# flexcompute/tidy3d

Measured on AMD Instinct MI355X. Metric: Mcells/s on 512^3 Yee grid, higher is better.
Workload: dtype f32; 1 GPU; v0: vacuum, PEC walls, curl stencil only; 512^3 Yee cells, Ez point dipole (GaussianPulse 200 THz), random +-1e-3 initial fields; parallelism=z-slab x1, bytes_per_cell_step=72

## Files before the change

### tidy3d_amd/csrc/fdtd_fused2.hpp

```cpp
#pragma once
#include "fdtd_kernels.hpp"

namespace fdtd {

constexpr int kMaxInj = 256;
struct InjP {
  int n;
  const int* start;
  const int4* ent;
  const float* val;
  const float* val2;
  int e2_in_sweep;
  float* cap;
  const int* dstart;
  const int* dlist;
  const struct DumpBox* dboxes;
  float* dump;
};
struct DumpBox {
  int lo0, lo1, lo2, nx, ny, nz;
  int off[6];
};
constexpr int kMaxDumps = 8;
struct DampT {
// ... 93 lines not shown
        if (!fused2_instantiated(fused2_lb(W, opt), opt)) return false;
        const int rep = fused2_opt(nt, mat, mon, clip, damp, disp, src, wv, true, W);
        if (!clip && fused2_rep_word(opt) && !fused2_instantiated(fused2_lb(W, rep), rep)) return false;
      }
    }
  return true;
}
static_assert(fused2_words_instantiated(), "fused2_opt forms a word that no list of instantiations holds");

#if !defined(FDTD_NO_EXJ)
#define FDTD_NO_EXJ 0
#endif
constexpr bool fused2_exj(int lb, int opt) { return !FDTD_NO_EXJ && (opt & kF2Damp) == 0 && !(lb == 512 && (opt & kF2Mat) != 0); }
constexpr int fused2_xch_arrays(int lb, int opt) {
  const int wv = fused2_whatif(opt);
  if (wv) return wv == 13 ? 9 : ((wv >= 10 && wv <= 12) ? 6 + (wv == 11 ? 2 : 3) : 8);
  return fused2_exj(lb, opt) ? 9 : 8;
}
constexpr size_t fused2_lds_bytes(int lb, int opt, int waves) {
  return ((size_t)fused2_xch_arrays(lb, opt) * waves * 64 + ((opt & kF2Damp) ? 2 * 64 : 0)) * sizeof(float4) + ((opt & kF2Mat) ? (size_t)kMaxMedia * sizeof(float2) : 0);
}
static_assert(fused2_lds_bytes(1024, kF2NT | kF2Mat | kF2Mon | kF2Clip | kF2Disp | kF2Src, 16) <= 160 * 1024 && fused2_lds_bytes(1024, kF2Mat | kF2Damp, 16) <= 160 * 1024 &&
              2 * fused2_lds_bytes(512, kF2NT, 8) <= 160 * 1024 && 2 * fused2_lds_bytes(512, kF2Mat | kF2Damp, 8) <= 160 * 1024,
              "fused2_step_kernel: LDS of a workgroup (two per CU for eight waves)");
constexpr bool fused2_lds_pinned(int lb, int opt) {
  const int wv = fused2_whatif(opt), w = lb / 64;
  if (wv) return fused2_lds_bytes(lb, opt, 16) == ((size_t)(wv == 13 ? 9 : ((wv >= 10 && wv <= 12) ? 6 + (wv == 11 ? 2 : 3) : 8)) * 16 * 64) * sizeof(float4);
  return fused2_lds_bytes(lb, opt, w) == ((size_t)(fused2_exj(lb, opt) ? 9 : 8) * w * 64 + ((opt & 8) ? 2 * 64 : 0)) * sizeof(float4) + ((opt & 2) ? (size_t)kMaxMedia * sizeof(float2) : 0);
}
#define FDTD_F2_X(LBV, OV) && fused2_lds_pinned(LBV, OV)
static_assert(true FDTD_F2_LIST_ALL(FDTD_F2_X), "fused2_lds_bytes: the LDS of a listed instantiation changed");
#undef FDTD_F2_X
constexpr int kMaxCap = 1024;
constexpr int kSeamArrays = 13;

void launch_inject_values(hipStream_t st, float* val, const float* w_re, const float* w_im, const float2* wave,
                          long long step, int n);
struct Fused2Launch {
  hipStream_t st;
  int waves, opt, grid_blocks;
  GridP g; FieldP a, b; StepP s; MatP m;
  int zchunk, nbx, nby, nbz, xcd_remap;
  InjP inj; float* seam; DampT dmp; ClipP clip; TileClassP tcl; DispP dp; SrcP sr;
};
#define FDTD_F2_ARGS(L) (L).g, (L).a, (L).b, (L).s, (L).m, (L).zchunk, (L).nbx, (L).nby, (L).nbz, (L).xcd_remap, (L).inj, (L).seam, (L).dmp, (L).clip, (L).tcl, (L).dp, (L).sr
#define FDTD_F2_CASE(LBV, OV)                                                                                                      \
  case fused2_key(LBV, OV):                                                                                                        \
    hipLaunchKernelGGL((fused2_step_kernel<LBV, OV>), dim3(L.grid_blocks, 1, 1), dim3(64, L.waves, 1), fused2_lds_bytes(LBV, OV, L.waves), L.st, \
                       FDTD_F2_ARGS(L));                                                                                           \
    return true;
#define FDTD_F2_LAUNCHER(NAME, LIST)                                                                                               \
  bool NAME(const Fused2Launch& L) {                                                                                               \
    switch (fused2_key(fused2_lb(L.waves, L.opt), L.opt)) { LIST(FDTD_F2_CASE) default: return false; }                            \
  }
bool launch_fused2_step(const Fused2Launch& L);
bool launch_fused2_step_src(const Fused2Launch& L);
bool launch_fused2_step_whatif(const Fused2Launch& L);
bool launch_fused2_step_disp(const Fused2Launch& L);
bool launch_fused2_step_clip(const Fused2Launch& L);
void launch_inject_table(hipStream_t st, float* tab, long long stride, long long off, const float* w_re, const float* w_im,
                         const float2* wave, long long n_steps, int n);
constexpr int kPairMons = 4;
struct PairRecP {
  int n_mon;
  int pre_done;
  BoxP box[kPairMons];
  int nc[kPairMons];
  int comp[kPairMons][6];
  int cap_off[kPairMons];
  float* out_n[kPairMons];
  float* out_m[kPairMons];
};
void launch_pair_record(hipStream_t st, const PairRecP& r, long long max_cells, const GridP& g, const FieldP& a, const FieldP& b,
                        const float* cap);
struct DftDumpP { int n; int slot[3]; int off[3]; };
void launch_dft_record_dump(hipStream_t st, const DftDumpP& r, const float* dump, float2* acc, long long cells, long long fstride,
                            const float2* phase, int nf);
void launch_seams(hipStream_t st, const GridP& g, const FieldP& b, const StepP& s, const MatP& m, const float* seam,
                  int n_seams, const DampT& dmp, const ClipP& clip, const InjP& inj, const SrcP& sr = SrcP{}, float* rep = nullptr);
constexpr int kRepArraysHost = 7;
inline size_t seam_scratch_floats(const GridP& g, int n_tiles_x) { return (size_t)n_tiles_x * kSeamArrays * (size_t)(g.nz + 2) * (size_t)g.ny; }
inline size_t seam_rep_floats(const GridP& g, int n_tiles_x) { return (size_t)n_tiles_x * kRepArraysHost * (size_t)g.nz * (size_t)g.ny; }
void launch_seam_flush(hipStream_t st, const GridP& g, const FieldP& b, const float* rep, int n_seams);

}
```

### tidy3d_amd/csrc/fdtd_kernels2.hpp

```cpp
#pragma once
#include "fdtd_fused2.hpp"

namespace fdtd {

__global__ __launch_bounds__(256) void pair_record_kernel(PairRecP r, GridP g, FieldP a, FieldP b, const float* cap) {
  const int mi = blockIdx.y / 6, ic = blockIdx.y % 6;
  if (mi >= r.n_mon || ic >= r.nc[mi]) return;
  const BoxP bx = r.box[mi];
  const long long cells = (long long)bx.nx * bx.ny * bx.nz;
  const long long t = (long long)blockIdx.x * blockDim.x + threadIdx.x;
  if (t >= cells) return;
  const int c = r.comp[mi][ic];
  const int lx = (int)(t % bx.nx), ly = (int)((t / bx.nx) % bx.ny), lz = (int)(t / ((long long)bx.nx * bx.ny));
  const long long p = (long long)(bx.lo2 + lz) * g.sxy + (long long)(bx.lo1 + ly) * g.nx + bx.lo0 + lx;
  const long long idx = (long long)ic * cells + t;
  const float* fa = c == 0 ? a.ex : (c == 1 ? a.ey : (c == 2 ? a.ez : (c == 3 ? a.hx : (c == 4 ? a.hy : a.hz))));
  const float* fb = c == 0 ? b.ex : (c == 1 ? b.ey : (c == 2 ? b.ez : (c == 3 ? b.hx : (c == 4 ? b.hy : b.hz))));
  const float mid = cap[r.cap_off[mi] + idx];
  float* on = r.out_n[mi];
  float* om = r.out_m[mi];
  if (c < 3) {
    if (on && !r.pre_done) on[idx] = 1.0f * fa[p];
    if (om) om[idx] = 1.0f * mid;
  } else {
// ... 6 lines not shown
                                                              long long fstride, const float2* phase, int nf) {
  const int q = blockIdx.y;
  const long long t = (long long)blockIdx.x * blockDim.x + threadIdx.x;
  if (t >= cells || q >= r.n) return;
  const float v = dump[r.off[q] + t];
  float2* a0 = acc + (long long)r.slot[q] * cells;
  for (int k = 0; k < nf; ++k) {
    const float2 ph = phase[k];
    float2 a = a0[(long long)k * fstride + t];
    a.x += v * ph.x;
    a.y += v * ph.y;
    a0[(long long)k * fstride + t] = a;
  }
}

__global__ __launch_bounds__(256) void inject_table_kernel(float* tab, long long stride, long long off, const float* w_re,
                                                           const float* w_im, const float2* wave, long long n_steps, int n) {
  const long long g = (long long)blockIdx.x * blockDim.x + threadIdx.x;
  if (g >= n_steps * n) return;
  const long long step = g / n;
  const int t = (int)(g % n);
  const float2 a = wave[step];
  tab[step * stride + off + t] = w_re[t] * a.x - w_im[t] * a.y;
}

__global__ __launch_bounds__(256) void inject_values_kernel(float* val, const float* w_re, const float* w_im,
                                                            const float2* wave, long long step, int n) {
  const int t = threadIdx.x;
  if (t >= n) return;
  const float2 a = wave[step];
  val[t] = w_re[t] * a.x - w_im[t] * a.y;
}

__device__ __forceinline__ long long seam_at(const GridP& g, int seam, int arr, int j, int k) {
  return (((long long)seam * kSeamArrays + arr) * (g.nz + 2) + (k + 1)) * g.ny + j;
}

constexpr int kRepArrays = 7;
__device__ __forceinline__ long long rep_base(const GridP& g, int n_tiles_x) {
  return (long long)n_tiles_x * kSeamArrays * (g.nz + 2) * g.ny;
}
__device__ __forceinline__ long long rep_at(const GridP& g, int seam, int arr, int j, int k) {
  return (((long long)seam * kRepArrays + arr) * g.nz + k) * g.ny + j;
}

__device__ __forceinline__ float lane_next(float v) {
#if defined(__HIP_DEVICE_COMPILE__)
  const int x = __builtin_bit_cast(int, v);
  return __builtin_bit_cast(float, __builtin_amdgcn_update_dpp(x, x, 0x130, 0xf, 0xf, false));
#else
  return __shfl_down(v, 1);
#endif
}
__device__ __forceinline__ float lane_prev(float v) {
#if defined(__HIP_DEVICE_COMPILE__)
  const int x = __builtin_bit_cast(int, v);
  return __builtin_bit_cast(float, __builtin_amdgcn_update_dpp(x, x, 0x138, 0xf, 0xf, false));
#else
  return __shfl_up(v, 1);
#endif
}

__device__ __forceinline__ void lds_dma16(const float* base, unsigned off, float4* dst, int lane) {
#if defined(__HIP_DEVICE_COMPILE__)
  const unsigned lds_addr = __builtin_amdgcn_readfirstlane((unsigned)(size_t)dst);
  unsigned keep;
  asm volatile("s_mov_b32 %0, m0\n\ts_mov_b32 m0, %2\n\ts_nop 0\n\tglobal_load_lds_dwordx4 %1, %3\n\ts_mov_b32 m0, %0"
               : "=&s"(keep) : "v"(off), "s"(lds_addr), "s"(base) : "memory");
#else
  dst[lane] = *reinterpret_cast<const float4*>(reinterpret_cast<const char*>(base) + off);
#endif
}
__device__ __forceinline__ void lds_dma_wait() {
// ... 154 lines not shown
    float ezx = lane_next(ezm[0]);
    if (act && (tx == 63 || last_x)) ezx = last_x ? (per_x ? a.ez[pb] : 0.f) : a.ez[pb + ux + V];
    const float ipz = s.ipz[kA - 1];
    ldf<V, true>(ho, uni(a.hx + pb), ubc);
    ldf<V, true>(hoy, uni(a.hy + pb), ubc);
    if constexpr (REP) {
      if (act && tx == 63 && !last_x) {
        const float* r = rpl + (long long)(kA - 1) * g.ny;
        hoy[V - 1] = r[0]; exm[V - 1] = r[2 * rep_arr]; eym[V - 1] = r[3 * rep_arr]; ezm[V - 1] = r[4 * rep_arr]; ezx = r[6 * rep_arr];
        if (use_jp) ezj[V - 1] = r[4 * rep_arr + 1];
      }
      if (xh) {
        const float* r = rpr + (long long)(kA - 1) * g.ny;
        eym[0] = r[5 * rep_arr]; ezm[0] = r[6 * rep_arr];
        if (use_jp) ezj[0] = r[6 * rep_arr + 1];
      }
    }
    if constexpr (DAMP) {
      const float czp = dmp.fc[2][kA - 1];
      const float4 b4 = xdm[tx], c4 = xdm[64 + tx];
      const float bx[V] = {b4.x, b4.y, b4.z, b4.w}, cx[V] = {c4.x, c4.y, c4.z, c4.w};
#pragma unroll
      for (int e = 0; e < V; ++e) { ho[e] *= bx[e] * cyv * czp; hoy[e] *= cx[e] * byv * czp; }
    }
#pragma unroll
    for (int e = 0; e < V; ++e) h1x[e] = upd_h(ho[e], ch, ezj[e] - ezm[e], ipy, eyk[e] - eym[e], ipz);
#pragma unroll
    for (int e = 0; e < V; ++e) {
      const float ez_ip = (e + 1 < V) ? ezm[(e + 1) % V] : ezx;
      h1y[e] = upd_h(hoy[e], ch, exk[e] - exm[e], ipz, ez_ip - ezm[e], ipx[e]);
    }
  }
  int cur = 0;
  const long long seam_arr = (long long)(g.nz + 2) * g.ny;
  const long long seam_row = seam_at(g, tile_x, 0, j, 0);
  struct Ld {
    float exn[V], eyn[V], ezk[V], exj[V], ezj[V], hxn[V], hyn[V], hzn[V];
    float eyx_g, ezx_g;
    float exn_m, ez_mm, ey_mm, ex_jm, hy_o, hz_o;
  };
  [[maybe_unused]] float4* pfb = xch + NXCH * slot;
  [[maybe_unused]] auto pf_issue = [&](int k) __attribute__((always_inline)) {
    if constexpr (PF != 0) {
      const long long pb = (long long)k * g.sxy + rowb;
      const long long up = (k < g.nz) ? g.sxy : 0;
      lds_dma_fence();
      if constexpr (PF == 10) {
        lds_dma16(uni(a.hx + pb), ubc, pfb + 0 * slot + ty * 64, tx);
        lds_dma16(uni(a.hy + pb), ubc, pfb + 1 * slot + ty * 64, tx);
        lds_dma16(uni(a.hz + pb), ubc, pfb + 2 * slot + ty * 64, tx);
      } else if constexpr (PF == 11) {
        lds_dma16(uni(a.ey + pb + up), ubc, pfb + 0 * slot + ty * 64, tx);
        lds_dma16(uni(a.hy + pb), ubc, pfb + 1 * slot + ty * 64, tx);
      } else {
        lds_dma16(uni(a.ex + pb + up), ubc, pfb + 0 * slot + ty * 64, tx);
        lds_dma16(uni(a.ey + pb + up), ubc, pfb + 1 * slot + ty * 64, tx);
        lds_dma16(uni(a.ez + pb), ubc, pfb + 2 * slot + ty * 64, tx);
      }
    }
  };
  [[maybe_unused]] auto pf_take = [&](int q, float (&o)[V]) __attribute__((always_inline)) {
    const float4 t4 = pfb[q * slot + me];
    o[0] = t4.x; o[1] = t4.y; o[2] = t4.z; o[3] = t4.w;
  };
  auto issue = [&](int k, Ld& L) __attribute__((always_inline)) {
    if constexpr (WHATIF == 3) {
      if (ty < 2 || ty == W - 1) {
        zero<V>(L.exn); zero<V>(L.eyn); zero<V>(L.ezk); zero<V>(L.exj); zero<V>(L.ezj); zero<V>(L.hxn); zero<V>(L.hyn); zero<V>(L.hzn);
// ... 60 lines not shown
            L.ezj[V - 1] = r[4 * rep_arr + 1];
            if (!EXJ || ty == W - 1 || k == kA) L.exj[V - 1] = r[2 * rep_arr + 1];
          }
        }
        if (xh) {
          const float* r = rpr + (long long)k * g.ny;
          L.ezk[0] = r[6 * rep_arr];
          if (up1) L.eyn[0] = r[5 * rep_arr + g.ny];
          if (use_jp) L.ezj[0] = r[6 * rep_arr + 1];
          if (do_e1) {
            L.exn_m = up1 ? r[2 * rep_arr + g.ny] : a.ex[pb + im + up];
            L.ez_mm = r[4 * rep_arr]; L.ey_mm = r[3 * rep_arr];
            if (use_jp) L.ex_jm = r[2 * rep_arr + 1];
            L.hy_o = r[0]; L.hz_o = r[rep_arr];
          }
        }
      }
    }
    if constexpr (PF != 0) {
      lds_dma_wait();
      if constexpr (PF == 10) { pf_take(0, L.hxn); pf_take(1, L.hyn); pf_take(2, L.hzn); }
      else if constexpr (PF == 11) { pf_take(0, L.eyn); pf_take(1, L.hyn); }
      else { pf_take(0, L.exn); pf_take(1, L.eyn); pf_take(2, L.ezk); }
    }
  };
  Ld LA, LB2;
  auto body = [&](int k, Ld& L) __attribute__((always_inline)) {
    const int txo = (MAT || DAMP) ? tx : opaque_lane(tx);
    const int i0o = (tile_x * 64 + txo) * V;
    const bool act = i0o < g.nx, last_x = i0o + V >= g.nx, first_x = i0o == 0;
    const bool xh = act && txo == 0 && (!first_x || per_x);
    [[maybe_unused]] const bool wall_x0 = first_x && !pmc_x0 && !per_x;
    const bool seam_l = (txo == 63 && !last_x) || (per_x && last_x), seam_r = txo == 0 && (tile_x > 0 || per_x);
    const long long seam_back = (tile_x > 0 ? -1 : (long long)(nbx - 1)) * kSeamArrays * seam_arr;
    const long long pb = (long long)k * g.sxy + rowb;
    const float ipz = s.ipz[k], idz = s.idz[k];
    [[maybe_unused]] float bzk = 1.f, czk = 1.f;
    if constexpr (DAMP) { bzk = dmp.fb[2][min(k, g.nz - 1)]; czk = dmp.fc[2][min(k, g.nz - 1)]; }
    int q0 = 0, q1 = 0;
    if (inj.n > 0) { q0 = inj.start[k]; q1 = inj.start[k + 1]; }
    [[maybe_unused]] int d0 = 0, d1 = 0;
    if constexpr (MON) { if (inj.dstart) { d0 = inj.dstart[k]; d1 = inj.dstart[k + 1]; } }
    float hy_m = 0.f, hz_m = 0.f;
    float (&exn)[V] = L.exn, (&eyn)[V] = L.eyn, (&ezk)[V] = L.ezk, (&exj)[V] = L.exj, (&ezj)[V] = L.ezj;
    float (&hxn)[V] = L.hxn, (&hyn)[V] = L.hyn, (&hzn)[V] = L.hzn;
    [[maybe_unused]] uint32_t rw = kBgWord;
    if constexpr (MAT) {
      if (do_e1) rw = m.roww[((long long)min(k, g.nz - 1) * g.ny + j) * nbx + tile_x];
    }
    [[maybe_unused]] int ss = -1;
    if constexpr (SRC) {
      if (do_e1 && k < g.nz) ss = sr.sseg[((long long)k * g.ny + j) * nbx + tile_x];
    }
    [[maybe_unused]] int ds = -1;
    if constexpr (DISP) {
      if (do_e1 && k < g.nz) ds = dp.dseg[((long long)k * g.ny + j) * nbx + tile_x];
    }
    if constexpr (WHATIF == 7) {
      issue(k, L);
      if (own && k > k0 && act) {
        const long long po = pb - g.sxy + i0;
        float o0[V], o1[V], o2[V];
#pragma unroll
        for (int e = 0; e < V; ++e) { o0[e] = L.exn[e] + L.exj[e]; o1[e] = L.ezk[e] + L.ezj[e]; o2[e] = L.eyn[e]; }
        stv_h<V, NT>(b.ex + po, o0); stv_h<V, NT>(b.ey + po, o2); stv_h<V, NT>(b.ez + po, o1);
        stv_h<V, NT>(b.hx + po, L.hxn); stv_h<V, NT>(b.hy + po, L.hyn); stv_h<V, NT>(b.hz + po, L.hzn);
      }
// ... 195 lines not shown
                  hit &= hit - 1;
                  const int d = lane_value(ev.x, l) - i0, c = lane_value(ev.z, l) - 8, w = lane_value(ev.w, l);
#pragma unroll
                  for (int e = 0; e < V; ++e)
                    if (d == e) inj.cap[w] = c == 0 ? e1xn[e] : (c == 1 ? e1yn[e] : e1zn[e]);
                }
              }
            }
          }
        }
        if constexpr (MON) {
          if (own && k >= k0 && k < k1) {
            for (int q = d0; q < d1; ++q) {
              const DumpBox bx = inj.dboxes[inj.dlist[q]];
              const int ly = j - bx.lo1, lz = k - bx.lo2;
              if (ly >= 0 && ly < bx.ny) {
                const long long rowo = ((long long)lz * bx.ny + ly) * bx.nx;
#pragma unroll
                for (int e = 0; e < V; ++e) {
                  const int lx = i0o + e - bx.lo0;
                  if (lx >= 0 && lx < bx.nx && act && (!CLIP || (i0o + e >= clip.i0 && i0o + e < clip.i1))) {
                    if (bx.off[0] >= 0) inj.dump[bx.off[0] + rowo + lx] = e1xn[e];
                    if (bx.off[1] >= 0) inj.dump[bx.off[1] + rowo + lx] = e1yn[e];
                    if (bx.off[2] >= 0) inj.dump[bx.off[2] + rowo + lx] = e1zn[e];
                    if (bx.off[3] >= 0) inj.dump[bx.off[3] + rowo + lx] = hxn[e];
                    if (bx.off[4] >= 0) inj.dump[bx.off[4] + rowo + lx] = hyn[e];
                    if (bx.off[5] >= 0) inj.dump[bx.off[5] + rowo + lx] = hzn[e];
                  }
                }
              }
            }
          }
        }
        if (WHATIF != 9 && (CLIP || (own && k >= k0 && k < k1)) && act) {
          float* sp = seam + seam_row + (long long)k * g.ny;
          if (seam_l) {
            sp[0] = hyn[V - 1];
            sp[seam_arr] = hzn[V - 1];
            sp[2 * seam_arr] = e1xn[V - 1];
            sp[3 * seam_arr] = e1yn[V - 1];
            sp[4 * seam_arr] = e1zn[V - 1];
          }
          if (seam_r) {
            sp[5 * seam_arr + seam_back] = e1yn[0];
            sp[6 * seam_arr + seam_back] = e1zn[0];
          }
        }
      }
    }
    float h2x[V], h2y[V], h2z[V];
    unspecified<V>(h2x); unspecified<V>(h2y); unspecified<V>(h2z);
    if (do_h2 && k > kA) {
      if constexpr (DAMP) {
        {
          const float4 b4 = xdm[tx];
          const float bx[V] = {b4.x, b4.y, b4.z, b4.w};
#pragma unroll
          for (int e = 0; e < V; ++e) h1x[e] *= bx[e] * cyv * cz_m;
        }
        {
          const float4 c4 = xdm[64 + tx];
          const float cx[V] = {c4.x, c4.y, c4.z, c4.w};
#pragma unroll
          for (int e = 0; e < V; ++e) { h1y[e] *= cx[e] * byv * cz_m; h1z[e] *= cx[e] * cyv * bz_m; }
        }
      }
      if constexpr (SRC) {
        if (ss_m >= 0 && act && sr.t->use_h2) {
          const long long qs = ((long long)ss_m * 3) * 256 + tx * V;
          float tx_[V], ty_[V], tz_[V];
          ldv<V>(tx_, sr.t->h2 + qs); ldv<V>(ty_, sr.t->h2 + qs + 256); ldv<V>(tz_, sr.t->h2 + qs + 512);
#pragma unroll
          for (int e = 0; e < V; ++e) { h1x[e] = h1x[e] + tx_[e]; h1y[e] = h1y[e] + ty_[e]; h1z[e] = h1z[e] + tz_[e]; }
          if (sr.t->h2b) {
            ldv<V>(tx_, sr.t->h2b + qs); ldv<V>(ty_, sr.t->h2b + qs + 256); ldv<V>(tz_, sr.t->h2b + qs + 512);
#pragma unroll
            for (int e = 0; e < V; ++e) { h1x[e] = h1x[e] + tx_[e]; h1y[e] = h1y[e] + ty_[e]; h1z[e] = h1z[e] + tz_[e]; }
          }
        }
// ... 11 lines not shown
              const float v = inj.val2[lane_value(ev.w, l)];
#pragma unroll
              for (int e = 0; e < V; ++e) {
                const bool mine = d == e;
                h1x[e] = (mine && code == 3) ? h1x[e] + v : h1x[e];
                h1y[e] = (mine && code == 4) ? h1y[e] + v : h1y[e];
                h1z[e] = (mine && code == 5) ? h1z[e] + v : h1z[e];
              }
            }
          }
        }
      }
      float eyx = lane_next(e1y[0]);
      float ezx = lane_next(e1z[0]);
      if (txo == 63 || last_x) { eyx = 0.f; ezx = 0.f; }
      float4 t0, t1;
      if constexpr (WHATIF == 6) {
        t0 = make_float4(e1x[0], e1x[1], e1x[2], e1x[3]); t1 = make_float4(e1z[0], e1z[1], e1z[2], e1z[3]);
      } else {
        t0 = xch[(4 + (E1S ? 0 : (cur ^ 1) * 2) + 0) * slot + me + 64];
        t1 = xch[(4 + (E1S ? 0 : (cur ^ 1) * 2) + 1) * slot + me + 64];
      }
      const float exj1[V] = {t0.x, t0.y, t0.z, t0.w}, ezj1[V] = {t1.x, t1.y, t1.z, t1.w};
#pragma unroll
      for (int e = 0; e < V; ++e) {
        const float ey_ip = (e + 1 < V) ? e1y[(e + 1) % V] : eyx;
        const float ez_ip = (e + 1 < V) ? e1z[(e + 1) % V] : ezx;
        h2x[e] = upd_h(h1x[e], ch, ezj1[e] - e1z[e], ipy, e1yn[e] - e1y[e], ipz_m);
        h2y[e] = upd_h(h1y[e], ch, e1xn[e] - e1x[e], ipz_m, ez_ip - e1z[e], ipx[e]);
        h2z[e] = upd_h(h1z[e], ch, ey_ip - e1y[e], ipx[e], exj1[e] - e1x[e], ipy);
      }
      if constexpr (CLIP) {
        if (act) {
          float* sq = seam + seam_row + (long long)(k - 1) * g.ny;
          if (seam_l) {
            sq[7 * seam_arr] = h2x[V - 1];
            sq[8 * seam_arr] = h2y[V - 2];
            sq[9 * seam_arr] = h2z[V - 2];
          }
          if (seam_r) {
            sq[10 * seam_arr + seam_back] = h2x[0];
            sq[11 * seam_arr + seam_back] = h2y[0];
            sq[12 * seam_arr + seam_back] = h2z[0];
          }
        }
      }
    }
    if constexpr (WHATIF != 6) {
      float4 t4;
      if constexpr (!E1S) {
        t4.x = e1xn[0]; t4.y = e1xn[1]; t4.z = e1xn[2]; t4.w = e1xn[3];
        xch[(4 + cur * 2 + 0) * slot + me] = t4;
        t4.x = e1zn[0]; t4.y = e1zn[1]; t4.z = e1zn[2]; t4.w = e1zn[3];
        xch[(4 + cur * 2 + 1) * slot + me] = t4;
      }
      if constexpr (EXJ) {
        t4.x = exn[0]; t4.y = exn[1]; t4.z = exn[2]; t4.w = exn[3];
        xch[XE * slot + me] = t4;
      }
      if constexpr (EZL) {
        if (k + 1 <= k1) {
          t4.x = ezn_pre[0]; t4.y = ezn_pre[1]; t4.z = ezn_pre[2]; t4.w = ezn_pre[3];
          xch[XZ * slot + me] = t4;
        }
      }
      t4.x = h2x[0]; t4.y = h2x[1]; t4.z = h2x[2]; t4.w = h2x[3];
      xch[2 * slot + me] = t4;
      t4.x = h2z[0]; t4.y = h2z[1]; t4.z = h2z[2]; t4.w = h2z[3];
      xch[3 * slot + me] = t4;
    }
    if constexpr (WHATIF != 2 && WHATIF != 6 && WHATIF != 8) __syncthreads();
    if constexpr (E1S) {
      float4 t4;
      t4.x = e1xn[0]; t4.y = e1xn[1]; t4.z = e1xn[2]; t4.w = e1xn[3];
      xch[4 * slot + me] = t4;
      t4.x = e1zn[0]; t4.y = e1zn[1]; t4.z = e1zn[2]; t4.w = e1zn[3];
// ... 77 lines not shown
          while (hit) {
            const int l = __ffsll(hit) - 1;
            hit &= hit - 1;
            const int d = lane_value(ev.x, l) - i0, code = lane_value(ev.z, l);
            const float v = inj.val2[lane_value(ev.w, l)];
#pragma unroll
            for (int e = 0; e < V; ++e) {
              if (d == e) {
                if (code == 0) ex[e] += v;
                else if (code == 1) ey[e] += v;
                else ez[e] += v;
              }
            }
          }
        }
      }
      if constexpr (DAMP) {
        if (dmp.e2) {
          {
            const float4 c4 = xdm[64 + tx];
            const float cx[V] = {c4.x, c4.y, c4.z, c4.w};
#pragma unroll
            for (int e = 0; e < V; ++e) ex[e] *= cx[e] * byv * bz_m;
          }
          {
            const float4 b4 = xdm[tx];
            const float bx[V] = {b4.x, b4.y, b4.z, b4.w};
#pragma unroll
            for (int e = 0; e < V; ++e) { ey[e] *= bx[e] * cyv * bz_m; ez[e] *= bx[e] * byv * cz_m; }
          }
        }
      }
      if (act && (!CLIP || (i0o >= clip.i0 && i0o < clip.i1))) {
        float* sq = seam + seam_row + (long long)(k - 1) * g.ny;
        if (!CLIP && WHATIF != 9 && txo == 63 && !last_x) {
          sq[7 * seam_arr] = h2x[V - 1];
          sq[8 * seam_arr] = h2y[V - 2];
          sq[9 * seam_arr] = h2z[V - 2];
        }
        if (!CLIP && WHATIF != 9 && txo == 0 && tile_x > 0) {
          sq[10 * seam_arr - kSeamArrays * seam_arr] = h2x[0];
          sq[11 * seam_arr - kSeamArrays * seam_arr] = h2y[0];
          sq[12 * seam_arr - kSeamArrays * seam_arr] = h2z[0];
        }
        const long long po = pb - g.sxy + i0;
        if (WHATIF != 5 || ex[0] == 3.0e38f) {
          stv_h<V, NT>(b.hx + po, h2x);
          stv_h<V, NT>(b.hy + po, h2y);
          stv_h<V, NT>(b.hz + po, h2z);
          stv_h<V, NT>(b.ex + po, ex);
          stv_h<V, NT>(b.ey + po, ey);
          stv_h<V, NT>(b.ez + po, ez);
        }
      }
    }
#pragma unroll
    for (int e = 0; e < V; ++e) {
      h2xm[e] = h2x[e]; h2ym[e] = h2y[e];
      h1x[e] = hxn[e]; h1y[e] = hyn[e]; h1z[e] = hzn[e];
      e1x[e] = e1xn[e]; e1y[e] = e1yn[e]; e1z[e] = e1zn[e];
      exk[e] = exn[e]; eyk[e] = eyn[e];
    }
    exk_m = L.exn_m;
    ipz_m = ipz; idz_m = idz;
    qm0 = q0; qm1 = q1;
    if constexpr (DAMP) { bz_m = bzk; cz_m = czk; }
    if constexpr (MAT) rw_m = rw;
    if constexpr (SRC) ss_m = ss;
    cur ^= 1;
  };
  if constexpr (PF != 0) pf_issue(kA);
  for (int k = kA; k <= k1; k += 2) {
    body(k, LA);
    if (k + 1 <= k1) body(k + 1, LB2);
  }
}
// ... 34 lines not shown
    const int G = xcd_remap, full = total / (8 * G) * (8 * G);
    if (t < full) {
      const int x = t & 7, mloc = t >> 3;
      t = ((mloc / G) * 8 + x) * G + mloc % G;
    }
    if (t >= total) return;
  }
  constexpr int OPTK = OPT | (fused2_exj(LB, OPT) ? 0 : kF2NoExj);
  if constexpr ((OPT & kF2Src) != 0) {
    if (tcl.cls && !(tcl.cls[t] & 4)) {
      fused2_tile_by_class<LB, (OPTK & ~kF2Src)>(g, a, b, s, m, zchunk, nbx, nby, nbz, inj, seam, dmp, clip, t, dp, sr, tcl);
      return;
    }
  }
  fused2_tile_by_class<LB, OPTK>(g, a, b, s, m, zchunk, nbx, nby, nbz, inj, seam, dmp, clip, t, dp, sr, tcl);
}

__global__ __launch_bounds__(256) void seam_kernel(GridP g, FieldP b, StepP s, MatP m,
                                                   const float* __restrict__ seam, int n_seams, DampT dmp, ClipP clip, InjP inj, SrcP sr,
                                                   float* __restrict__ rep) {
  const long long t = (long long)blockIdx.x * blockDim.x + threadIdx.x;
  const int nj = clip.j1 - clip.j0;
  const long long per = (long long)nj * (clip.k1 - clip.k0);
  if (t >= per * n_seams) return;
  const int sm = (int)(t / per);
  const int k = clip.k0 + (int)((t % per) / nj), j = clip.j0 + (int)(t % nj);
  const bool wrap = g.bcx0 == BC_PERIODIC && sm == n_seams - 1;
  const int c = wrap ? g.nx : (sm + 1) * 256;
  const int cc = wrap ? 0 : c;
  const bool wl = c - 1 >= clip.i0 && c - 1 < clip.i1, wr = cc >= clip.i0 && cc < clip.i1;
  if (!wl && !wr) return;
  const float ch = g.ch;
  const float ipx = s.ipx[c - 1];
  auto A = [&](int a, int jj, int kk) { return seam[seam_at(g, sm, a, jj, kk)]; };
  auto h2 = [&](int jj, int kk, float& hy, float& hz) {
    const float e1x = A(2, jj, kk), e1y = A(3, jj, kk), e1z = A(4, jj, kk);
    const float e1x_jp = (jj + 1 < g.ny) ? A(2, jj + 1, kk) : 0.f;
    float h1y = A(0, jj, kk), h1z = A(1, jj, kk);
    if (dmp.fb[0]) {
      const float cxv = dmp.fc[0][c - 1];
      h1y *= cxv * dmp.fb[1][jj] * dmp.fc[2][kk];
      h1z *= cxv * dmp.fc[1][jj] * dmp.fb[2][kk];
    }
    if (sr.sseg && sr.t->use_h2) {
      const int blk = sr.sseg[((long long)kk * g.ny + jj) * ((g.nx + 255) >> 8) + ((c - 1) >> 8)];
      if (blk >= 0) {
        const long long qs = ((long long)blk * 3) * 256 + ((c - 1) & 255);
        h1y = h1y + sr.t->h2[qs + 256];
        h1z = h1z + sr.t->h2[qs + 512];
        if (sr.t->h2b) { h1y = h1y + sr.t->h2b[qs + 256]; h1z = h1z + sr.t->h2b[qs + 512]; }
      }
    }
    hy = upd_h(h1y, ch, A(2, jj, kk + 1) - e1x, s.ipz[kk], A(6, jj, kk) - e1z, ipx);
    hz = upd_h(h1z, ch, A(5, jj, kk) - e1y, ipx, e1x_jp - e1x, s.ipy[jj]);
  };
  float hy_m, hz_m;
  h2(j, k, hy_m, hz_m);
  const bool pmc_y0 = g.bcy0 == BC_PMC, pmc_z0 = !g.pec_z0;
  const bool wall_y = (j == 0) && !pmc_y0, wall_z = (k == 0) && !pmc_z0;
  const bool mir_y = (j == 0) && pmc_y0, mir_z = (k == 0) && pmc_z0;
  const long long pr = (long long)k * g.sxy + (long long)j * g.nx;
  const long long p = pr + cc, pl = pr + c - 1;
  if (!rep && wl) { b.hy[pl] = hy_m; b.hz[pl] = hz_m; }
  const float idy = s.idy[j], idz = s.idz[k], idx_m = s.idx[c - 1], idx_c = s.idx[cc];
  const float hx_m = A(7, j, k), hy_mm = A(8, j, k), hz_mm = A(9, j, k);
  const float hx_c = A(10, j, k), hy_c = A(11, j, k), hz_c = A(12, j, k);
  auto coef = [&](long long cell, int c) {
    return m.m4 ? m.lut[(m.m4[cell] >> (10 * c)) & 1023u] : make_float2(m.ca1, m.cb1);
  };
  float ex_m = 0.f, ey_m = 0.f, ez_m = 0.f, ey_c = 0.f, ez_c = 0.f;
  float hy_k = 0.f, hz_j = 0.f, dum;
  if (mir_z) hy_k = -hy_m; else if (!wall_z) h2(j, k - 1, hy_k, dum);
  if (mir_y) hz_j = -hz_m; else if (!wall_y) h2(j - 1, k, dum, hz_j);
  const float hxm_k = wall_z ? 0.f : (mir_z ? -hx_m : A(7, j, k - 1)), hxc_k = wall_z ? 0.f : (mir_z ? -hx_c : A(10, j, k - 1));
  const float hxm_j = wall_y ? 0.f : (mir_y ? -hx_m : A(7, j - 1, k)), hxc_j = wall_y ? 0.f : (mir_y ? -hx_c : A(10, j - 1, k));
  if (!wall_y && !wall_z) { const float2 q = coef(pl, 0); ex_m = upd_e(A(2, j, k), q.x, q.y, hz_m - hz_j, idy, hy_m - hy_k, idz); }
  if (!wall_z) {
    const float2 qm = coef(pl, 1), qc = coef(p, 1);
    ey_m = upd_e(A(3, j, k), qm.x, qm.y, hx_m - hxm_k, idz, hz_m - hz_mm, idx_m);
    ey_c = upd_e(A(5, j, k), qc.x, qc.y, hx_c - hxc_k, idz, hz_c - hz_m, idx_c);
  }
  if (!wall_y) {
    const float2 qm = coef(pl, 2), qc = coef(p, 2);
    ez_m = upd_e(A(4, j, k), qm.x, qm.y, hy_m - hy_mm, idx_m, hx_m - hxm_j, idy);
    ez_c = upd_e(A(6, j, k), qc.x, qc.y, hy_c - hy_m, idx_c, hx_c - hxc_j, idy);
  }
  if (sr.sseg && sr.t->use_e2) {
    const int nbxg = (g.nx + 255) >> 8;
    const int bl = sr.sseg[((long long)k * g.ny + j) * nbxg + ((c - 1) >> 8)], br = sr.sseg[((long long)k * g.ny + j) * nbxg + (cc >> 8)];
    if (bl >= 0) {
      const long long qs = ((long long)bl * 3) * 256 + ((c - 1) & 255);
      ex_m = ex_m + sr.t->e2[qs]; ey_m = ey_m + sr.t->e2[qs + 256]; ez_m = ez_m + sr.t->e2[qs + 512];
      if (sr.t->e2b) { ex_m = ex_m + sr.t->e2b[qs]; ey_m = ey_m + sr.t->e2b[qs + 256]; ez_m = ez_m + sr.t->e2b[qs + 512]; }
    }
    if (br >= 0) {
      const long long qs = ((long long)br * 3) * 256 + (cc & 255);
      ey_c = ey_c + sr.t->e2[qs + 256]; ez_c = ez_c + sr.t->e2[qs + 512];
      if (sr.t->e2b) { ey_c = ey_c + sr.t->e2b[qs + 256]; ez_c = ez_c + sr.t->e2b[qs + 512]; }
    }
  }
  if (inj.val2 && inj.e2_in_sweep) {
    const int q0 = inj.start[k], q1 = inj.start[k + 1];
    for (int q = q0; q < q1; ++q) {
      const int4 en = inj.ent[q];
      if (en.y != j || en.z >= 3) continue;
      const float v = inj.val2[en.w];
      if (en.x == c - 1) { if (en.z == 0) ex_m += v; else if (en.z == 1) ey_m += v; else ez_m += v; }
      else if (en.x == cc) { if (en.z == 1) ey_c += v; else if (en.z == 2) ez_c += v; }
    }
  }
  if (dmp.fb[0] && dmp.e2) {
    const float bxm = dmp.fb[0][c - 1], cxm = dmp.fc[0][c - 1], bxc = dmp.fb[0][cc];
    const float byv = dmp.fb[1][j], cyv = dmp.fc[1][j], bzv = dmp.fb[2][k], czv = dmp.fc[2][k];
    ex_m *= cxm * byv * bzv; ey_m *= bxm * cyv * bzv; ez_m *= bxm * byv * czv;
    ey_c *= bxc * cyv * bzv; ez_c *= bxc * byv * czv;
  }
  if (rep) {
    float* r = rep + rep_at(g, sm, 0, j, k);
// ... 22 lines not shown
```

Measured before the change: 205,600 Mcells/s.

## Interleave seam scratch arrays into 16-float rows with vectorized stores and loads

Changes the seam scratch buffer from 13 separate planar arrays to an interleaved layout of one 16-float row per (seam, k, j). The main kernel writes seam values with float4 stores, and the seam fixup kernel reads each cell's data with four float4 loads instead of many scattered scalar loads. Configurations with monitors, dispersion or sources keep scalar stores through an opaque stride. The aim is fewer memory transactions in the seam path, at the cost of a somewhat larger scratch buffer and more code paths.

```diff
diff --git a/tidy3d_amd/csrc/fdtd_fused2.hpp b/tidy3d_amd/csrc/fdtd_fused2.hpp
--- a/tidy3d_amd/csrc/fdtd_fused2.hpp
+++ b/tidy3d_amd/csrc/fdtd_fused2.hpp
@@ -149,7 +149,7 @@
 static_assert(true FDTD_F2_LIST_ALL(FDTD_F2_X), "fused2_lds_bytes: the LDS of a listed instantiation changed");
 #undef FDTD_F2_X
 constexpr int kMaxCap = 1024;
-constexpr int kSeamArrays = 13;
+constexpr int kSeamRow = 16;
 
 void launch_inject_values(hipStream_t st, float* val, const float* w_re, const float* w_im, const float2* wave,
                           long long step, int n);
@@ -196,7 +196,7 @@
 void launch_seams(hipStream_t st, const GridP& g, const FieldP& b, const StepP& s, const MatP& m, const float* seam,
                   int n_seams, const DampT& dmp, const ClipP& clip, const InjP& inj, const SrcP& sr = SrcP{}, float* rep = nullptr);
 constexpr int kRepArraysHost = 7;
-inline size_t seam_scratch_floats(const GridP& g, int n_tiles_x) { return (size_t)n_tiles_x * kSeamArrays * (size_t)(g.nz + 2) * (size_t)g.ny; }
+inline size_t seam_scratch_floats(const GridP& g, int n_tiles_x) { return (size_t)n_tiles_x * (size_t)(g.nz + 2) * (size_t)g.ny * kSeamRow; }
 inline size_t seam_rep_floats(const GridP& g, int n_tiles_x) { return (size_t)n_tiles_x * kRepArraysHost * (size_t)g.nz * (size_t)g.ny; }
 void launch_seam_flush(hipStream_t st, const GridP& g, const FieldP& b, const float* rep, int n_seams);
 
diff --git a/tidy3d_amd/csrc/fdtd_kernels2.hpp b/tidy3d_amd/csrc/fdtd_kernels2.hpp
--- a/tidy3d_amd/csrc/fdtd_kernels2.hpp
+++ b/tidy3d_amd/csrc/fdtd_kernels2.hpp
@@ -62,13 +62,25 @@
   val[t] = w_re[t] * a.x - w_im[t] * a.y;
 }
 
-__device__ __forceinline__ long long seam_at(const GridP& g, int seam, int arr, int j, int k) {
-  return (((long long)seam * kSeamArrays + arr) * (g.nz + 2) + (k + 1)) * g.ny + j;
+__device__ __forceinline__ long long seam_at(const GridP& g, int seam, int j, int k) {
+  return ((((long long)seam * (g.nz + 2)) + (k + 1)) * g.ny + j) * kSeamRow;
+}
+__device__ __forceinline__ void seam_st4(float* p, float x, float y, float z, float w) {
+  *reinterpret_cast<float4*>(p) = make_float4(x, y, z, w);
+}
+template <int SLOT>
+__device__ __forceinline__ void seam_st1(float* row, long long one, float v) { row[SLOT * one] = v; }
+__device__ __forceinline__ int opaque_one() {
+  int v = 1;
+#if defined(__HIP_DEVICE_COMPILE__)
+  asm volatile("" : "+s"(v));
+#endif
+  return v;
 }
 
 constexpr int kRepArrays = 7;
 __device__ __forceinline__ long long rep_base(const GridP& g, int n_tiles_x) {
-  return (long long)n_tiles_x * kSeamArrays * (g.nz + 2) * g.ny;
+  return (long long)n_tiles_x * (g.nz + 2) * g.ny * kSeamRow;
 }
 __device__ __forceinline__ long long rep_at(const GridP& g, int seam, int arr, int j, int k) {
   return (((long long)seam * kRepArrays + arr) * g.nz + k) * g.ny + j;
@@ -289,8 +301,11 @@
     }
   }
   int cur = 0;
-  const long long seam_arr = (long long)(g.nz + 2) * g.ny;
-  const long long seam_row = seam_at(g, tile_x, 0, j, 0);
+  constexpr bool H1MOD = DAMP || SRC || MON || CLIP;
+  constexpr bool NARROW = MON || DISP || SRC || (CLIP && MAT) || WHATIF == 4 || WHATIF == 5 || PF != 0;
+  const long long seam_pl = (long long)g.ny * kSeamRow;
+  [[maybe_unused]] const long long seam_one = NARROW ? opaque_one() : 1;
+  const long long seam_row = seam_at(g, tile_x, j, 0);
   struct Ld {
     float exn[V], eyn[V], ezk[V], exj[V], ezj[V], hxn[V], hyn[V], hzn[V];
     float eyx_g, ezx_g;
@@ -417,7 +432,7 @@
     const bool xh = act && txo == 0 && (!first_x || per_x);
     [[maybe_unused]] const bool wall_x0 = first_x && !pmc_x0 && !per_x;
     const bool seam_l = (txo == 63 && !last_x) || (per_x && last_x), seam_r = txo == 0 && (tile_x > 0 || per_x);
-    const long long seam_back = (tile_x > 0 ? -1 : (long long)(nbx - 1)) * kSeamArrays * seam_arr;
+    const long long seam_back = (tile_x > 0 ? -1 : (long long)(nbx - 1)) * (g.nz + 2) * seam_pl;
     const long long pb = (long long)k * g.sxy + rowb;
     const float ipz = s.ipz[k], idz = s.idz[k];
     [[maybe_unused]] float bzk = 1.f, czk = 1.f;
@@ -679,19 +694,18 @@
             }
           }
         }
-        if (WHATIF != 9 && (CLIP || (own && k >= k0 && k < k1)) && act) {
-          float* sp = seam + seam_row + (long long)k * g.ny;
-          if (seam_l) {
-            sp[0] = hyn[V - 1];
-            sp[seam_arr] = hzn[V - 1];
-            sp[2 * seam_arr] = e1xn[V - 1];
-            sp[3 * seam_arr] = e1yn[V - 1];
-            sp[4 * seam_arr] = e1zn[V - 1];
-          }
-          if (seam_r) {
-            sp[5 * seam_arr + seam_back] = e1yn[0];
-            sp[6 * seam_arr + seam_back] = e1zn[0];
-          }
+        if constexpr (NARROW) {
+          if (WHATIF != 9 && (CLIP || (own && k >= k0 && k < k1)) && act) {
+            float* sp = seam + seam_row + k * seam_pl;
+            if (seam_l) {
+              seam_st1<0>(sp, seam_one, hyn[V - 1]); seam_st1<1>(sp, seam_one, hzn[V - 1]);
+              seam_st1<2>(sp, seam_one, e1xn[V - 1]); seam_st1<3>(sp, seam_one, e1yn[V - 1]); seam_st1<4>(sp, seam_one, e1zn[V - 1]);
+            }
+            if (seam_r) { seam_st1<8>(sp + seam_back, seam_one, e1yn[0]); seam_st1<9>(sp + seam_back, seam_one, e1zn[0]); }
+          }
+        } else if constexpr (H1MOD) {
+          if (WHATIF != 9 && (CLIP || (own && k >= k0 && k < k1)) && act && seam_l)
+            seam_st4(seam + seam_row + k * seam_pl, hyn[V - 1], hzn[V - 1], e1xn[V - 1], e1yn[V - 1]);
         }
       }
     }
@@ -769,16 +783,16 @@
       }
       if constexpr (CLIP) {
         if (act) {
-          float* sq = seam + seam_row + (long long)(k - 1) * g.ny;
-          if (seam_l) {
-            sq[7 * seam_arr] = h2x[V - 1];
-            sq[8 * seam_arr] = h2y[V - 2];
-            sq[9 * seam_arr] = h2z[V - 2];
-          }
-          if (seam_r) {
-            sq[10 * seam_arr + seam_back] = h2x[0];
-            sq[11 * seam_arr + seam_back] = h2y[0];
-            sq[12 * seam_arr + seam_back] = h2z[0];
+          float* sq = seam + seam_row + (k - 1) * seam_pl;
+          if constexpr (NARROW) {
+            if (seam_l) { seam_st1<5>(sq, seam_one, h2x[V - 1]); seam_st1<6>(sq, seam_one, h2y[V - 2]); seam_st1<7>(sq, seam_one, h2z[V - 2]); }
+            if (seam_r) { seam_st1<10>(sq + seam_back, seam_one, h2x[0]); seam_st1<11>(sq + seam_back, seam_one, h2y[0]); seam_st1<12>(sq + seam_back, seam_one, h2z[0]); }
+          } else {
+            if (seam_l) seam_st4(sq + 4, e1z[V - 1], h2x[V - 1], h2y[V - 2], h2z[V - 2]);
+            if (seam_r) {
+              seam_st4(sq + seam_back + 8, e1y[0], e1z[0], h2x[0], h2y[0]);
+              sq[seam_back + 12] = h2z[0];
+            }
           }
         }
       }
@@ -922,16 +936,20 @@
         }
       }
       if (act && (!CLIP || (i0o >= clip.i0 && i0o < clip.i1))) {
-        float* sq = seam + seam_row + (long long)(k - 1) * g.ny;
+        float* sq = seam + seam_row + (k - 1) * seam_pl;
         if (!CLIP && WHATIF != 9 && txo == 63 && !last_x) {
-          sq[7 * seam_arr] = h2x[V - 1];
-          sq[8 * seam_arr] = h2y[V - 2];
-          sq[9 * seam_arr] = h2z[V - 2];
+          if constexpr (NARROW) { seam_st1<5>(sq, seam_one, h2x[V - 1]); seam_st1<6>(sq, seam_one, h2y[V - 2]); seam_st1<7>(sq, seam_one, h2z[V - 2]); }
+          else {
+            if constexpr (!H1MOD) seam_st4(sq, h1y[V - 1], h1z[V - 1], e1x[V - 1], e1y[V - 1]);
+            seam_st4(sq + 4, e1z[V - 1], h2x[V - 1], h2y[V - 2], h2z[V - 2]);
+          }
         }
         if (!CLIP && WHATIF != 9 && txo == 0 && tile_x > 0) {
-          sq[10 * seam_arr - kSeamArrays * seam_arr] = h2x[0];
-          sq[11 * seam_arr - kSeamArrays * seam_arr] = h2y[0];
-          sq[12 * seam_arr - kSeamArrays * seam_arr] = h2z[0];
+          if constexpr (NARROW) { seam_st1<10>(sq + seam_back, seam_one, h2x[0]); seam_st1<11>(sq + seam_back, seam_one, h2y[0]); seam_st1<12>(sq + seam_back, seam_one, h2z[0]); }
+          else {
+            seam_st4(sq + seam_back + 8, e1y[0], e1z[0], h2x[0], h2y[0]);
+            sq[seam_back + 12] = h2z[0];
+          }
         }
         const long long po = pb - g.sxy + i0;
         if (WHATIF != 5 || ex[0] == 3.0e38f) {
@@ -1032,11 +1050,11 @@
   if (!wl && !wr) return;
   const float ch = g.ch;
   const float ipx = s.ipx[c - 1];
-  auto A = [&](int a, int jj, int kk) { return seam[seam_at(g, sm, a, jj, kk)]; };
-  auto h2 = [&](int jj, int kk, float& hy, float& hz) {
-    const float e1x = A(2, jj, kk), e1y = A(3, jj, kk), e1z = A(4, jj, kk);
-    const float e1x_jp = (jj + 1 < g.ny) ? A(2, jj + 1, kk) : 0.f;
-    float h1y = A(0, jj, kk), h1z = A(1, jj, kk);
+  auto P = [&](int jj, int kk, int q) { return *reinterpret_cast<const float4*>(seam + seam_at(g, sm, jj, kk) + 4 * q); };
+  const float4 r0 = P(j, k, 0), r1 = P(j, k, 1), r2 = P(j, k, 2), r3 = P(j, k, 3);
+  auto h2 = [&](int jj, int kk, const float4& q0, const float4& q1, const float4& q2, float e1x_kp, float e1x_jp, float& hy, float& hz) {
+    const float e1x = q0.z, e1y = q0.w, e1z = q1.x;
+    float h1y = q0.x, h1z = q0.y;
     if (dmp.fb[0]) {
       const float cxv = dmp.fc[0][c - 1];
       h1y *= cxv * dmp.fb[1][jj] * dmp.fc[2][kk];
@@ -1051,11 +1069,11 @@
         if (sr.t->h2b) { h1y = h1y + sr.t->h2b[qs + 256]; h1z = h1z + sr.t->h2b[qs + 512]; }
       }
     }
-    hy = upd_h(h1y, ch, A(2, jj, kk + 1) - e1x, s.ipz[kk], A(6, jj, kk) - e1z, ipx);
-    hz = upd_h(h1z, ch, A(5, jj, kk) - e1y, ipx, e1x_jp - e1x, s.ipy[jj]);
+    hy = upd_h(h1y, ch, e1x_kp - e1x, s.ipz[kk], q2.y - e1z, ipx);
+    hz = upd_h(h1z, ch, q2.x - e1y, ipx, e1x_jp - e1x, s.ipy[jj]);
   };
   float hy_m, hz_m;
-  h2(j, k, hy_m, hz_m);
+  h2(j, k, r0, r1, r2, P(j, k + 1, 0).z, (j + 1 < g.ny) ? P(j + 1, k, 0).z : 0.f, hy_m, hz_m);
   const bool pmc_y0 = g.bcy0 == BC_PMC, pmc_z0 = !g.pec_z0;
   const bool wall_y = (j == 0) && !pmc_y0, wall_z = (k == 0) && !pmc_z0;
   const bool mir_y = (j == 0) && pmc_y0, mir_z = (k == 0) && pmc_z0;
@@ -1063,27 +1081,36 @@
   const long long p = pr + cc, pl = pr + c - 1;
   if (!rep && wl) { b.hy[pl] = hy_m; b.hz[pl] = hz_m; }
   const float idy = s.idy[j], idz = s.idz[k], idx_m = s.idx[c - 1], idx_c = s.idx[cc];
-  const float hx_m = A(7, j, k), hy_mm = A(8, j, k), hz_mm = A(9, j, k);
-  const float hx_c = A(10, j, k), hy_c = A(11, j, k), hz_c = A(12, j, k);
+  const float hx_m = r1.y, hy_mm = r1.z, hz_mm = r1.w;
+  const float hx_c = r2.z, hy_c = r2.w, hz_c = r3.x;
   auto coef = [&](long long cell, int c) {
     return m.m4 ? m.lut[(m.m4[cell] >> (10 * c)) & 1023u] : make_float2(m.ca1, m.cb1);
   };
   float ex_m = 0.f, ey_m = 0.f, ez_m = 0.f, ey_c = 0.f, ez_c = 0.f;
   float hy_k = 0.f, hz_j = 0.f, dum;
-  if (mir_z) hy_k = -hy_m; else if (!wall_z) h2(j, k - 1, hy_k, dum);
-  if (mir_y) hz_j = -hz_m; else if (!wall_y) h2(j - 1, k, dum, hz_j);
-  const float hxm_k = wall_z ? 0.f : (mir_z ? -hx_m : A(7, j, k - 1)), hxc_k = wall_z ? 0.f : (mir_z ? -hx_c : A(10, j, k - 1));
-  const float hxm_j = wall_y ? 0.f : (mir_y ? -hx_m : A(7, j - 1, k)), hxc_j = wall_y ? 0.f : (mir_y ? -hx_c : A(10, j - 1, k));
-  if (!wall_y && !wall_z) { const float2 q = coef(pl, 0); ex_m = upd_e(A(2, j, k), q.x, q.y, hz_m - hz_j, idy, hy_m - hy_k, idz); }
+  float hxm_k = 0.f, hxc_k = 0.f, hxm_j = 0.f, hxc_j = 0.f;
+  if (mir_z) { hy_k = -hy_m; hxm_k = -hx_m; hxc_k = -hx_c; }
+  else if (!wall_z) {
+    const float4 q0 = P(j, k - 1, 0), q1 = P(j, k - 1, 1), q2 = P(j, k - 1, 2);
+    h2(j, k - 1, q0, q1, q2, r0.z, (j + 1 < g.ny) ? P(j + 1, k - 1, 0).z : 0.f, hy_k, dum);
+    hxm_k = q1.y; hxc_k = q2.z;
+  }
+  if (mir_y) { hz_j = -hz_m; hxm_j = -hx_m; hxc_j = -hx_c; }
+  else if (!wall_y) {
+    const float4 q0 = P(j - 1, k, 0), q1 = P(j - 1, k, 1), q2 = P(j - 1, k, 2);
+    h2(j - 1, k, q0, q1, q2, P(j - 1, k + 1, 0).z, r0.z, dum, hz_j);
+    hxm_j = q1.y; hxc_j = q2.z;
+  }
+  if (!wall_y && !wall_z) { const float2 q = coef(pl, 0); ex_m = upd_e(r0.z, q.x, q.y, hz_m - hz_j, idy, hy_m - hy_k, idz); }
   if (!wall_z) {
     const float2 qm = coef(pl, 1), qc = coef(p, 1);
-    ey_m = upd_e(A(3, j, k), qm.x, qm.y, hx_m - hxm_k, idz, hz_m - hz_mm, idx_m);
-    ey_c = upd_e(A(5, j, k), qc.x, qc.y, hx_c - hxc_k, idz, hz_c - hz_m, idx_c);
+    ey_m = upd_e(r0.w, qm.x, qm.y, hx_m - hxm_k, idz, hz_m - hz_mm, idx_m);
+    ey_c = upd_e(r2.x, qc.x, qc.y, hx_c - hxc_k, idz, hz_c - hz_m, idx_c);
   }
   if (!wall_y) {
     const float2 qm = coef(pl, 2), qc = coef(p, 2);
-    ez_m = upd_e(A(4, j, k), qm.x, qm.y, hy_m - hy_mm, idx_m, hx_m - hxm_j, idy);
-    ez_c = upd_e(A(6, j, k), qc.x, qc.y, hy_c - hy_m, idx_c, hx_c - hxc_j, idy);
+    ez_m = upd_e(r1.x, qm.x, qm.y, hy_m - hy_mm, idx_m, hx_m - hxm_j, idy);
+    ez_c = upd_e(r2.y, qc.x, qc.y, hy_c - hy_m, idx_c, hx_c - hxc_j, idy);
   }
   if (sr.sseg && sr.t->use_e2) {
     const int nbxg = (g.nx + 255) >> 8;
```

After: 210,700 Mcells/s (median of 6 runs). 2.5% higher.
